# dylkot/cNMF

Measured on AMD Instinct MI355X. Metric: NMF restarts/sec (50000x2000xK5..13), higher is better.
Workload: dtype f32 (exact integer f16 plane x 2 f16 planes with per-row exponent, f32 accumulate)

## Files before the change

### cnmf_amd/csrc/kernels_gemm2h.hip.h

```cpp
#pragma once
#include <hip/hip_runtime.h>
#include "kernels_gemm3.hip.h"

namespace cnmf {

typedef _Float16 f16x8 __attribute__((ext_vector_type(8)));
typedef float f32x4_g __attribute__((ext_vector_type(4)));
#ifdef CNMF_G2_LDS_STORE
constexpr bool G2_LDS_STORE = true;
#else
constexpr bool G2_LDS_STORE = false;
#endif

constexpr int G2_ROWB = 64;
constexpr int G2_A = G3_MW * G2_ROWB;
constexpr int G2_B = G3C_JW * 32;
constexpr float G2_COUNT_BASE = 2048.0f;

constexpr int g2_imgs(int nsub) { return nsub == 1 ? 4 : 3; }
constexpr int g2_img_bytes(int nsub, bool with_hi) { return nsub * (G2_A + (with_hi ? 2 : 1) * G2_B); }
constexpr int g2_lds_bytes(int nsub, bool with_hi) { return g2_imgs(nsub) * g2_img_bytes(nsub, with_hi); }

__device__ __forceinline__ unsigned short f16_bits(float x)
{
    const _Float16 h = (_Float16)x;
    return __builtin_bit_cast(unsigned short, h);
}
__device__ __forceinline__ float f16_to_f32(unsigned short b) { return (float)__builtin_bit_cast(_Float16, b); }

__device__ __forceinline__ int g2_row_shift(float mx)
{
    if (!(mx > 0.f)) return 0;
    int e;
    frexpf(mx, &e);
    const int s = 15 - e;
    return s > 120 ? 120 : (s < -110 ? -110 : s);
}

__device__ __forceinline__ void split2h(float y, unsigned short& h, unsigned short& m)
{
    h = f16_bits(y);
    m = f16_bits(y - f16_to_f32(h));
}

struct SplitFused { const int* shift_in; int* shift_out; };
template <int TROWS, int TKB>
__device__ __forceinline__ void split2h_tiled_body(const float* __restrict__ src, int ld, int K, int TR,
                                                   unsigned short* __restrict__ dst, const double* __restrict__ kscale,
                                                   const float* __restrict__ rmax_part, int parts,
                                                   float* __restrict__ inv_scale, int bx, int nbx, int by,
                                                   unsigned short* tile_, float* red_, SplitFused fu = SplitFused{nullptr, nullptr})
{
    static_assert(TROWS * TKB == 256, "tile = 256 (row, block) pairs");
    constexpr int NQ = 256 / TROWS;
    constexpr int KQ = TKB * 4;
    constexpr int RPP = 256 / KQ;
    unsigned short (*tile)[TROWS][32] = reinterpret_cast<unsigned short (*)[TROWS][32]>(tile_);
    float (*red)[TROWS] = reinterpret_cast<float (*)[TROWS]>(red_);
    const int t = threadIdx.x;
    const int r0 = by * TROWS;
    const int kq = t % KQ, rr = t / KQ;
    const int ntiles = K / (16 * TKB);
    const bool fused = fu.shift_in != nullptr;
    float4 v[4];
    if (!fused) {
        const int k0 = bx * 16 * TKB;
#pragma unroll
        for (int i = 0; i < 4; ++i)
            v[i] = *reinterpret_cast<const float4*>(src + (size_t)(r0 + rr + RPP * i) * ld + k0 + kq * 4);
    }
    {
        const int row = t % TROWS, qt = t / TROWS;
        float mx = 0.f;
        for (int p0 = qt; p0 < parts; p0 += 8 * NQ) {
            float v[8];
#pragma unroll
            for (int j = 0; j < 8; ++j) v[j] = (p0 + j * NQ < parts) ? rmax_part[(size_t)(r0 + row) * parts + p0 + j * NQ] : 0.f;
#pragma unroll
            for (int j = 0; j < 8; ++j) mx = fmaxf(mx, v[j]);
        }
        red[qt][row] = mx;
    }
    __syncthreads();
    int sh[4];
    bool redo = false;
#pragma unroll
    for (int i = 0; i < 4; ++i) {
        const int row = rr + RPP * i;
        float mx = 0.f;
#pragma unroll
        for (int q = 0; q < NQ; ++q) mx = fmaxf(mx, red[q][row]);
        sh[i] = g2_row_shift(mx);
        if (fused) {
            const int su = fu.shift_in[r0 + row];
            const float ymax = ldexpf(mx, su);
            const bool ok = !(mx > 0.f) || (ymax < 60000.0f && ymax >= 1024.0f);
            const bool keep = !(mx > 0.f) || (ymax < 46340.0f && ymax >= 8192.0f);
            if (bx == 0 && kq == 0) fu.shift_out[r0 + row] = (ok && keep) ? su : sh[i];
            if (ok) sh[i] = su; else redo = true;
        }
        if (bx == 0 && kq == 0) inv_scale[r0 + row] = ldexpf(1.0f, -sh[i]);
    }
    if (fused) {
        if (!__syncthreads_or(redo ? 1 : 0)) return;
        const int k0 = bx * 16 * TKB;
#pragma unroll
        for (int i = 0; i < 4; ++i)
            v[i] = *reinterpret_cast<const float4*>(src + (size_t)(r0 + rr + RPP * i) * ld + k0 + kq * 4);
    }
    __syncthreads();
    const int Kb = K / 16;
    const int tr = r0 / TR, rin = r0 % TR;
    for (int kt = bx; kt < ntiles; kt += nbx) {
        const int k0 = kt * 16 * TKB;
        float4 vn[4];
        const bool has_next = kt + nbx < ntiles;
        if (has_next) {
#pragma unroll
            for (int i = 0; i < 4; ++i)
                vn[i] = *reinterpret_cast<const float4*>(src + (size_t)(r0 + rr + RPP * i) * ld + (k0 + nbx * 16 * TKB) + kq * 4);
        }
#pragma unroll
        for (int i = 0; i < 4; ++i) {
            const int row = rr + RPP * i;
            float x[4] = {v[i].x, v[i].y, v[i].z, v[i].w};
            if (kscale) {
#pragma unroll
                for (int e = 0; e < 4; ++e) x[e] = (float)((double)x[e] * kscale[k0 + kq * 4 + e]);
            }
            unsigned short p[2][4];
#pragma unroll
            for (int e = 0; e < 4; ++e) split2h(ldexpf(x[e], sh[i]), p[0][e], p[1][e]);
            const int hf = (kq >> 1) & 1, swz = (row >> 2) & 3;
#pragma unroll
            for (int q = 0; q < 2; ++q) {
                uint2 w;
                w.x = p[q][0] | ((unsigned)p[q][1] << 16); w.y = p[q][2] | ((unsigned)p[q][3] << 16);
                *reinterpret_cast<uint2*>(&tile[kq >> 2][row][((2 * q + hf) ^ swz) * 8 + (kq & 1) * 4]) = w;
            }
        }
        __syncthreads();
#pragma unroll
        for (int pass = 0; pass < 4; ++pass) {
            const int c = pass * 256 + t;
            const int b = c / (TROWS * 4), within = c % (TROWS * 4);
            unsigned short* g = dst + (((size_t)tr * Kb + (k0 / 16 + b)) * TR + rin) * 32;
            reinterpret_cast<u32x4*>(g)[within] = reinterpret_cast<const u32x4*>(&tile[b][0][0])[within];
        }
        __syncthreads();
        if (has_next) {
#pragma unroll
            for (int i = 0; i < 4; ++i) v[i] = vn[i];
        }
    }
}

template <int TROWS, int TKB>
__global__ __launch_bounds__(256) void split2h_tiled_kernel(const float* __restrict__ src, int ld, int K, int TR,
                                                            unsigned short* __restrict__ dst,
                                                            const double* __restrict__ kscale,
                                                            const float* __restrict__ rmax_part, int parts,
                                                            float* __restrict__ inv_scale)
{
    __shared__ __attribute__((aligned(16))) unsigned short tile[256 * 32];
    float* red = reinterpret_cast<float*>(tile);
    split2h_tiled_body<TROWS, TKB>(src, ld, K, TR, dst, kscale, rmax_part, parts, inv_scale, blockIdx.x, gridDim.x,
                                   blockIdx.y, tile, red);
}

__global__ __launch_bounds__(256) void rowmax_part_kernel(const float* __restrict__ V, int ld, int L, int span,
                                                          const double* __restrict__ kscale, int parts,
                                                          float* __restrict__ rmax_part)
{
    const int row = blockIdx.y * 4 + (threadIdx.x >> 6), lane = threadIdx.x & 63, p = blockIdx.x;
    const int j0 = p * span, j1 = min(L, j0 + span);
    float mx = 0.f;
    for (int j = j0 + lane; j < j1; j += 64) {
        float x = V[(size_t)row * ld + j];
        if (kscale) x = (float)((double)x * kscale[j]);
        mx = fmaxf(mx, x);
    }
#pragma unroll
    for (int o = 32; o > 0; o >>= 1) mx = fmaxf(mx, __shfl_xor(mx, o, 64));
    if (lane == 0) rmax_part[(size_t)row * parts + p] = mx;
}

__device__ __forceinline__ void count_lo_hi_2048(float n, float& lo, float& hi)
{
    if (n <= G2_COUNT_BASE) { lo = n; hi = 0.f; }
    else { hi = floorf(n * (1.0f / G2_COUNT_BASE)); lo = n - G2_COUNT_BASE * hi; hi *= G2_COUNT_BASE; }
}

__device__ __forceinline__ void store_plane_row_swz(unsigned short* d, const unsigned short* p, int row_in_tile)
{
    const int swz = (row_in_tile >> 3) & 1;
#pragma unroll
    for (int hf = 0; hf < 2; ++hf) {
        u32x4 w;
        w.x = p[8 * hf + 0] | ((unsigned)p[8 * hf + 1] << 16); w.y = p[8 * hf + 2] | ((unsigned)p[8 * hf + 3] << 16);
        w.z = p[8 * hf + 4] | ((unsigned)p[8 * hf + 5] << 16); w.w = p[8 * hf + 6] | ((unsigned)p[8 * hf + 7] << 16);
        *reinterpret_cast<u32x4*>(d + (hf ^ swz) * 8) = w;
    }
}

__global__ __launch_bounds__(256) void count_planes_f16_kernel(const float* __restrict__ X, int ld, int N, int G,
                                                               int rows_pad, int K, int TR,
                                                               const float* __restrict__ unit,
                                                               unsigned short* __restrict__ dst,
                                                               unsigned short* __restrict__ dst_hi,
                                                               unsigned int* __restrict__ hiflag)
{
    const long long t = (long long)blockIdx.x * 256 + threadIdx.x;
    const int Kb = K / 16;
    if (t >= (long long)rows_pad * Kb) return;
    const int row = (int)(t / Kb), kb = (int)(t % Kb);
    unsigned short p[16], ph[16];
    bool any_hi = false;
#pragma unroll
    for (int i = 0; i < 16; ++i) {
        const int g = kb * 16 + i;
        float n = 0.f, lo, hi;
        if (row < N && g < G) { const float u = unit[g]; if (u > 0.f) n = rintf(X[(size_t)row * ld + g] / u); }
        count_lo_hi_2048(n, lo, hi);
        p[i] = f16_bits(lo); ph[i] = f16_bits(hi);
        any_hi |= hi != 0.f;
    }
    const size_t blk = (size_t)(row / TR) * Kb + kb;
    store_plane_row_swz(dst + (blk * TR + (row % TR)) * 16, p, row % TR);
    if (dst_hi) {
        store_plane_row_swz(dst_hi + (blk * TR + (row % TR)) * 16, ph, row % TR);
        if (any_hi) atomicOr(&hiflag[(size_t)(row / TR) * ((Kb + 31) / 32) + (kb >> 5)], 1u << (kb & 31));
    }
}

__global__ __launch_bounds__(256) void count_planes_f16_transpose_kernel(const float* __restrict__ X, int ld, int N, int G,
                                                                         int rows_pad, int K, int TR,
                                                                         const float* __restrict__ unit,
                                                                         unsigned short* __restrict__ dst,
                                                                         unsigned short* __restrict__ dst_hi,
                                                                         unsigned int* __restrict__ hiflag)
{
    const int j = blockIdx.y * 256 + threadIdx.x;
    const int kb = blockIdx.x;
    if (j >= rows_pad) return;
    const int Kb = K / 16;
    const float u = (j < G) ? unit[j] : 0.f;
    unsigned short p[16], ph[16];
    bool any_hi = false;
#pragma unroll
    for (int i = 0; i < 16; ++i) {
        const int c = kb * 16 + i;
        float n = 0.f, lo, hi;
        if (u > 0.f && c < N) n = rintf(X[(size_t)c * ld + j] / u);
        count_lo_hi_2048(n, lo, hi);
        p[i] = f16_bits(lo); ph[i] = f16_bits(hi);
        any_hi |= hi != 0.f;
    }
    const size_t blk = (size_t)(j / TR) * Kb + kb;
    store_plane_row_swz(dst + (blk * TR + (j % TR)) * 16, p, j % TR);
    if (dst_hi) {
        store_plane_row_swz(dst_hi + (blk * TR + (j % TR)) * 16, ph, j % TR);
        if (any_hi) atomicOr(&hiflag[(size_t)(j / TR) * ((Kb + 31) / 32) + (kb >> 5)], 1u << (kb & 31));
    }
}

__global__ __launch_bounds__(256) void x2h_rowshift_kernel(const float* __restrict__ X, int ld, int N, int G,
                                                           int transpose, int rows_pad, int* __restrict__ shift,
                                                           float* __restrict__ inv_scale)
{
    if (!transpose) {
        const int row = blockIdx.x * 4 + (threadIdx.x >> 6), lane = threadIdx.x & 63;
        if (row >= rows_pad) return;
        float mx = 0.f;
        if (row < N) for (int g = lane; g < G; g += 64) mx = fmaxf(mx, X[(size_t)row * ld + g]);
#pragma unroll
        for (int o = 32; o > 0; o >>= 1) mx = fmaxf(mx, __shfl_xor(mx, o, 64));
        if (lane == 0) { const int s = g2_row_shift(mx); shift[row] = s; inv_scale[row] = ldexpf(1.0f, -s); }
    } else {
        const int g = blockIdx.x * 256 + threadIdx.x;
        if (g >= rows_pad) return;
        float mx = 0.f;
        if (g < G) for (int r = 0; r < N; ++r) mx = fmaxf(mx, X[(size_t)r * ld + g]);
        const int s = g2_row_shift(mx);
        shift[g] = s; inv_scale[g] = ldexpf(1.0f, -s);
    }
}

__global__ __launch_bounds__(256) void x2h_planes_kernel(const float* __restrict__ X, int ld, int N, int G, int rows_pad,
                                                         int K, int TR, const int* __restrict__ shift,
                                                         unsigned short* __restrict__ dst_h, unsigned short* __restrict__ dst_m)
{
    const long long t = (long long)blockIdx.x * 256 + threadIdx.x;
    const int Kb = K / 16;
    if (t >= (long long)rows_pad * Kb) return;
    const int row = (int)(t / Kb), kb = (int)(t % Kb);
    const int s = shift[row];
    unsigned short ph[16], pm[16];
#pragma unroll
    for (int i = 0; i < 16; ++i) {
        const int g = kb * 16 + i;
        const float x = (row < N && g < G) ? X[(size_t)row * ld + g] : 0.f;
        split2h(ldexpf(x, s), ph[i], pm[i]);
    }
    const size_t blk = (size_t)(row / TR) * Kb + kb;
    store_plane_row_swz(dst_h + (blk * TR + (row % TR)) * 16, ph, row % TR);
    store_plane_row_swz(dst_m + (blk * TR + (row % TR)) * 16, pm, row % TR);
}

__global__ __launch_bounds__(256) void x2h_planes_transpose_kernel(const float* __restrict__ X, int ld, int N, int G,
                                                                   int rows_pad, int K, int TR,
                                                                   const int* __restrict__ shift,
                                                                   unsigned short* __restrict__ dst_h,
                                                                   unsigned short* __restrict__ dst_m)
{
    const int j = blockIdx.y * 256 + threadIdx.x;
    const int kb = blockIdx.x;
    if (j >= rows_pad) return;
    const int Kb = K / 16;
    const int s = shift[j];
    unsigned short ph[16], pm[16];
#pragma unroll
    for (int i = 0; i < 16; ++i) {
        const int c = kb * 16 + i;
        const float x = (j < G && c < N) ? X[(size_t)c * ld + j] : 0.f;
        split2h(ldexpf(x, s), ph[i], pm[i]);
    }
    const size_t blk = (size_t)(j / TR) * Kb + kb;
    store_plane_row_swz(dst_h + (blk * TR + (j % TR)) * 16, ph, j % TR);
    store_plane_row_swz(dst_m + (blk * TR + (j % TR)) * 16, pm, j % TR);
}

__global__ __launch_bounds__(256) void count_max_base_kernel(const float* __restrict__ X, int ld, int N, int G,
                                                             const float* __restrict__ unit, float base,
                                                             unsigned* __restrict__ any_big)
{
    const int g = blockIdx.x * 256 + threadIdx.x;
    if (g >= G) return;
    const float u = unit[g];
    if (u <= 0.f) return;
    const int r0 = blockIdx.y * 256, r1 = min(N, r0 + 256);
    bool big = false;
    for (int r = r0; r < r1; ++r) big |= rintf(X[(size_t)r * ld + g] / u) > base;
    if (big) atomicOr(any_big, 1u);
}

struct G2NoEpi { static constexpr bool enabled = false; };
template <int NSUB, bool HI, int VAR = 0, bool NTB = true, bool PART = false, bool GEN = false, class EPI = G2NoEpi>
__device__ __forceinline__ void gemm2h_segment(const unsigned char* __restrict__ A2, const unsigned char* __restrict__ B1,
                                               const unsigned char* __restrict__ Bhi,
                                               const unsigned int* __restrict__ hiflag,
                                               const float* __restrict__ rscale,
                                               int Kb, float* __restrict__ C, int ldc, int m0, int j0, int kb0,
                                               int nkb, unsigned char* smem, const float* __restrict__ cscale = nullptr,
                                               unsigned live = 0xffu, const EPI* epi = nullptr, bool whole_tile = false)
{
    constexpr int IMGS = g2_imgs(NSUB);
    constexpr int IMG = g2_img_bytes(NSUB, HI);
    constexpr int OFF_B = NSUB * G2_A;
    constexpr int OFF_H = OFF_B + NSUB * G2_B;
    constexpr int NA = NSUB * 2, NB = NSUB;
    constexpr int NDMA = NA + NB;
    const int tid = threadIdx.x;
    const int lane = tid & 63, wave = tid >> 6;
    const int grp = wave >> 2, wn = wave & 3;
    const int li = lane & 31, h = lane >> 5;
    const int nst = nkb / NSUB;
    const unsigned lv = PART ? (unsigned)__builtin_amdgcn_readfirstlane((int)((live >> (grp * 4)) & 0xfu)) : 0xfu;
#define G2_LIVE(m_) (!PART || ((lv >> (m_)) & 1u))

    const size_t jblk = ((size_t)(j0 / G3C_JW) * Kb + kb0);
    const unsigned char* abase = A2 + ((size_t)(m0 / G3_MW) * Kb + kb0) * G2_A + tid * 16;
    const unsigned char* bbase = B1 + jblk * G2_B + tid * 16;
    const unsigned char* hbase = HI ? Bhi + jblk * G2_B + tid * 16 : nullptr;
    unsigned int fw[5] = {0u, 0u, 0u, 0u, 0u};
    if (HI) {
        const int KW = (Kb + 31) >> 5, w0 = kb0 >> 5;
        const unsigned int* fr = hiflag + (size_t)(j0 / G3C_JW) * KW;
#pragma unroll
        for (int w = 0; w < 5; ++w)
            fw[w] = (nkb > 129) ? 0xFFFFFFFFu : ((w0 + w < KW) ? __builtin_amdgcn_readfirstlane(fr[w0 + w]) : 0u);
    }
    const int fbit0 = kb0 & 31;

    f32x16_3 acc[4][2];
#pragma unroll
    for (int m = 0; m < 4; ++m)
#pragma unroll
        for (int n = 0; n < 2; ++n)
#pragma unroll
            for (int r = 0; r < 16; ++r) acc[m][n][r] = 0.f;

    const int a_row = (grp * 128 + li) * G2_ROWB;
    const int a_s0 = ((0 + h) ^ ((li >> 2) & 3)) * 16, a_s1 = ((2 + h) ^ ((li >> 2) & 3)) * 16;
    const int b_off = OFF_B + (wn * 64 + li) * 32 + (h ^ ((li >> 3) & 1)) * 16;

#define G2_BLKFLAG(b_) (HI && ((fw[(fbit0 + (b_)) >> 5 > 4 ? 4 : (fbit0 + (b_)) >> 5] >> ((fbit0 + (b_)) & 31)) & 1u))
#define G2_ISSUE(s_)                                                                               \
    {                                                                                              \
        unsigned char* d_ = smem + ((s_) % IMGS) * IMG + wave * 1024;                              \
        const unsigned char* a_ = abase + (size_t)(s_) * (NSUB * G2_A);                            \
        _Pragma("unroll") for (int i = 0; i < NA; ++i)                                             \
            __builtin_amdgcn_global_load_lds(G3_AS1(a_ + i * 8192), G3_AS3(d_ + i * 8192), 16, 0, 0); \
                                        \
        _Pragma("unroll") for (int i = 0; i < NB; ++i)                                             \
            __builtin_amdgcn_global_load_lds(G3_AS1(bbase + (size_t)(s_) * (NSUB * G2_B) + i * 8192), \
                                             G3_AS3(d_ + OFF_B + i * 8192), 16, 0, NTB ? 2 : 0);   \
        if (HI) {                                                                                  \
            _Pragma("unroll") for (int i = 0; i < NB; ++i)                                         \
                if (G2_BLKFLAG((s_) * NSUB + i))                                                   \
                    __builtin_amdgcn_global_load_lds(G3_AS1(hbase + (size_t)(s_) * (NSUB * G2_B) + i * 8192), \
                                                     G3_AS3(d_ + OFF_H + i * 8192), 16, 0, NTB ? 2 : 0); \
        }                                                                                          \
    }
#define G2_FRAG(ptr_) __builtin_bit_cast(f16x8, *reinterpret_cast<const u32x4*>(ptr_))
#define G2_READ(s_)                                                                                \
    {                                                                                              \
        const unsigned char* bb = smem + ((s_) % IMGS) * IMG;                                      \
        _Pragma("unroll") for (int u = 0; u < NSUB; ++u) {                                         \
            _Pragma("unroll") for (int n = 0; n < 2; ++n) bq[u][n] = G2_FRAG(bb + b_off + u * G2_B + n * 32 * 32); \
            if (HI) { _Pragma("unroll") for (int n = 0; n < 2; ++n)                                \
                          bh[u][n] = G2_FRAG(bb + b_off + NSUB * G2_B + u * G2_B + n * 32 * 32); } \
            _Pragma("unroll") for (int m = 0; m < 4; ++m) {                                        \
                aq[u][m][0] = G2_FRAG(bb + u * G2_A + a_row + m * 32 * G2_ROWB + a_s0);            \
                aq[u][m][1] = G2_FRAG(bb + u * G2_A + a_row + m * 32 * G2_ROWB + a_s1);            \
            }                                                                                      \
        }                                                                                          \
        __builtin_amdgcn_sched_barrier(0);                                                         \
    }
#define G2_MFMA(b_, u_, m_, q_)                                                                    \
    if (G2_LIVE(m_)) {                                                                             \
    acc[m_][0] = __builtin_amdgcn_mfma_f32_32x32x16_f16(aq[u_][m_][q_], b_[u_][0], acc[m_][0], 0, 0, 0); \
    acc[m_][1] = __builtin_amdgcn_mfma_f32_32x32x16_f16(aq[u_][m_][q_], b_[u_][1], acc[m_][1], 0, 0, 0); }
#define G2_MFMA4(b_, u_, ma_, mb_)                                                                 \
    G2_MFMA(b_, u_, ma_, 1) G2_MFMA(b_, u_, mb_, 1) G2_MFMA(b_, u_, ma_, 0) G2_MFMA(b_, u_, mb_, 0)
#define G2_MFMA2H(b_, u_, ma_, mb_) G2_MFMA(b_, u_, ma_, 0) G2_MFMA(b_, u_, mb_, 0)
#define G2_HALF(ma_, mb_)                                                                          \
    _Pragma("unroll") for (int u = 0; u < NSUB; ++u) {                                             \
        G2_MFMA4(bq, u, ma_, mb_)                                                                  \
        if (HI) { if (hi_blk[u]) { if constexpr (GEN) { G2_MFMA2H(bh, u, ma_, mb_) } else { G2_MFMA4(bh, u, ma_, mb_) } } } \
    }
#define G2_WAIT_AHEAD(cnt_)                                                                        \
    {                                                                                              \
        if constexpr ((cnt_) * NDMA == 0) G3_WAIT_VM(0);                                           \
        else if constexpr ((cnt_) * NDMA == 3) G3_WAIT_VM(3);                                      \
        else if constexpr ((cnt_) * NDMA == 6) G3_WAIT_VM(6);                                      \
        else if constexpr ((cnt_) * NDMA == 12) G3_WAIT_VM(12);                                    \
        else G3_WAIT_VM(0);                                                                        \
    }

    f16x8 bq[NSUB][2], bh[NSUB][2], aq[NSUB][4][2];
    constexpr int AHEAD = IMGS - 1;
    constexpr bool SPREAD = VAR >= 1 && NSUB == 2 && !HI;
    constexpr bool SPREADG = VAR >= 1 && NSUB == 1 && ((HI && GEN) || !HI);
    constexpr bool PRIO = false;
    constexpr bool NOMFMA = VAR == 2, NODMA = VAR == 3 || VAR == 6 || VAR == 7, SPLITRD = VAR >= 4;
    static_assert(VAR != 1 && VAR != 5, "instruction streams 1 and 5 were retired");
    constexpr bool NOREAD = VAR == 6 || VAR == 7;
    constexpr bool NOBAR = VAR == 7;
    G3_WAIT_VM(0);
    G2_ISSUE(0)
    if (nst > 1) G2_ISSUE(1)
    if (AHEAD > 2 && nst > 2) G2_ISSUE(2)
    if (AHEAD > 2 && nst > 2) G2_WAIT_AHEAD(2) else if (nst > 1) G2_WAIT_AHEAD(1) else G2_WAIT_AHEAD(0)
    if (grp == 1) G3_RAW_BARRIER()
    if constexpr (SPREADG) {
        static_assert(!SPREADG || (IMGS == 4 && NA == 2 && NB == 1), "one-block spread stream: four images, pieces A0 A1 B (Bhi)");
#define G2G_PIECE(s_, i_)                                                                          \
        {                                                                                          \
            unsigned char* d_ = smem + ((s_) % IMGS) * IMG + wave * 1024;                          \
            if ((i_) < NA)                                                                         \
                __builtin_amdgcn_global_load_lds(G3_AS1(abase + (size_t)(s_) * G2_A + (i_) * 8192), \
                                                 G3_AS3(d_ + (i_) * 8192), 16, 0, 0);              \
            else if ((i_) == NA)                                                                   \
                __builtin_amdgcn_global_load_lds(G3_AS1(bbase + (size_t)(s_) * G2_B), G3_AS3(d_ + OFF_B), 16, 0, NTB ? 2 : 0); \
            else if constexpr (HI)                                                                 \
                __builtin_amdgcn_global_load_lds(G3_AS1(hbase + (size_t)(s_) * G2_B), G3_AS3(d_ + OFF_H), 16, 0, NTB ? 2 : 0); \
            __builtin_amdgcn_sched_barrier(0);                                                     \
        }
#define G2G_READ_A(s_)                                                                             \
        {                                                                                          \
            const unsigned char* bb = smem + ((s_) % IMGS) * IMG;                                  \
            _Pragma("unroll") for (int n = 0; n < 2; ++n) bq[0][n] = G2_FRAG(bb + b_off + n * 32 * 32); \
            _Pragma("unroll") for (int m = 0; m < 2; ++m) {                                        \
                aq[0][m][1] = G2_FRAG(bb + a_row + m * 32 * G2_ROWB + a_s1);                       \
                aq[0][m][0] = G2_FRAG(bb + a_row + m * 32 * G2_ROWB + a_s0);                       \
            }                                                                                      \
            if constexpr (HI) { _Pragma("unroll") for (int n = 0; n < 2; ++n) bh[0][n] = G2_FRAG(bb + b_off + G2_B + n * 32 * 32); } \
            __builtin_amdgcn_sched_barrier(0);                                                     \
        }
#define G2G_READ_B(s_)                                                                             \
        {                                                                                          \
            const unsigned char* bb = smem + ((s_) % IMGS) * IMG;                                  \
            _Pragma("unroll") for (int m = 2; m < 4; ++m) {                                        \
                aq[0][m][1] = G2_FRAG(bb + a_row + m * 32 * G2_ROWB + a_s1);                       \
                aq[0][m][0] = G2_FRAG(bb + a_row + m * 32 * G2_ROWB + a_s0);                       \
            }                                                                                      \
            __builtin_amdgcn_sched_barrier(0);                                                     \
        }
#define G2G_STEP(MORE_)                                                                            \
        {                                                                                          \
            G3_RAW_BARRIER()                                         \
            G2G_READ_A(s)                                                                          \
            G2_MFMA(bq, 0, 0, 1) G2_MFMA(bq, 0, 1, 1)                                              \
            if (MORE_) G2G_PIECE(s + AHEAD, 0)                                                     \
            G2_MFMA(bq, 0, 0, 0) G2_MFMA(bq, 0, 1, 0)                                              \
            G2G_READ_B(s)                                                                          \
            if (MORE_) G2G_PIECE(s + AHEAD, 1)                                                     \
            if constexpr (HI) { G2_MFMA(bh, 0, 0, 0) G2_MFMA(bh, 0, 1, 0) }                        \
            asm volatile("s_waitcnt lgkmcnt(0)" ::: "memory");                                     \
             \
            if (s + 1 < nst) { if (MORE_) { if constexpr (HI) G3_WAIT_VM(6); else G3_WAIT_VM(5); } else G3_WAIT_VM(0); } \
            G3_RAW_BARRIER()                                                              \
            G2_MFMA(bq, 0, 2, 1) G2_MFMA(bq, 0, 3, 1)                                              \
            if (MORE_) G2G_PIECE(s + AHEAD, 2)                                                     \
            G2_MFMA(bq, 0, 2, 0) G2_MFMA(bq, 0, 3, 0)                                              \
            if constexpr (HI) { if (MORE_) G2G_PIECE(s + AHEAD, 3)                                 \
                                G2_MFMA(bh, 0, 2, 0) G2_MFMA(bh, 0, 3, 0) }                        \
        }
        {
            int s = 0;
            const int n_main = nst - AHEAD;
            for (; s < n_main; ++s) G2G_STEP(true)
            for (; s < nst; ++s) G2G_STEP(false)
        }
#undef G2G_STEP
#undef G2G_READ_B
#undef G2G_READ_A
#undef G2G_PIECE
    } else if constexpr (!SPREAD) {
        for (int s = 0; s < nst; ++s) {
            bool hi_blk[NSUB];
#pragma unroll
            for (int u = 0; u < NSUB; ++u) hi_blk[u] = G2_BLKFLAG(s * NSUB + u);
            G3_RAW_BARRIER()
            if (s + AHEAD < nst) G2_ISSUE(s + AHEAD)
            G2_READ(s)
            if (PRIO) __builtin_amdgcn_s_setprio(1);
            G2_HALF(0, 1)
            if (PRIO) __builtin_amdgcn_s_setprio(0);
            asm volatile("s_waitcnt lgkmcnt(0)" ::: "memory");
            if (s + 1 < nst) {
                if (AHEAD > 2 && s + 3 < nst) G2_WAIT_AHEAD(2) else if (s + 2 < nst) G2_WAIT_AHEAD(1) else G2_WAIT_AHEAD(0)
            }
            G3_RAW_BARRIER()
            if (PRIO) __builtin_amdgcn_s_setprio(1);
            G2_HALF(2, 3)
            if (PRIO) __builtin_amdgcn_s_setprio(0);
        }
    } else {
#define G2_PIECE(s_, i_)                                                                           \
        {                                                                                          \
            unsigned char* d_ = smem + ((s_) % IMGS) * IMG + wave * 1024;                          \
            if ((i_) < NA)                                                                         \
                __builtin_amdgcn_global_load_lds(G3_AS1(abase + (size_t)(s_) * (NSUB * G2_A) + (i_) * 8192), \
                                                 G3_AS3(d_ + (i_) * 8192), 16, 0, 0);              \
            else                                                                                   \
                __builtin_amdgcn_global_load_lds(G3_AS1(bbase + (size_t)(s_) * (NSUB * G2_B) + ((i_) - NA) * 8192), \
                                                 G3_AS3(d_ + OFF_B + ((i_) - NA) * 8192), 16, 0, NTB ? 2 : 0); \
            __builtin_amdgcn_sched_barrier(0);                                                     \
        }
#define G2_MF(u_, m_, q_)                                                                          \
        if constexpr (NOMFMA) { asm volatile("" :: "v"(aq[u_][m_][q_]), "v"(bq[u_][0]), "v"(bq[u_][1])); }        \
        else { G2_MFMA(bq, u_, m_, q_) }
#define G2_READ_A(s_)                                                                              \
    {                                                                                              \
        const unsigned char* bb = smem + ((s_) % IMGS) * IMG;                                      \
        _Pragma("unroll") for (int u = 0; u < NSUB; ++u) {                                         \
            _Pragma("unroll") for (int n = 0; n < 2; ++n) bq[u][n] = G2_FRAG(bb + b_off + u * G2_B + n * 32 * 32); \
            _Pragma("unroll") for (int m = 0; m < 2; ++m) {                                        \
                aq[u][m][1] = G2_FRAG(bb + u * G2_A + a_row + m * 32 * G2_ROWB + a_s1);            \
                aq[u][m][0] = G2_FRAG(bb + u * G2_A + a_row + m * 32 * G2_ROWB + a_s0);            \
            }                                                                                      \
        }                                                                                          \
        __builtin_amdgcn_sched_barrier(0);                                                         \
    }
#define G2_READ_B(s_)                                                                              \
    {                                                                                              \
        const unsigned char* bb = smem + ((s_) % IMGS) * IMG;                                      \
        _Pragma("unroll") for (int u = 0; u < NSUB; ++u)                                           \
            _Pragma("unroll") for (int m = 2; m < 4; ++m) {                                        \
                aq[u][m][1] = G2_FRAG(bb + u * G2_A + a_row + m * 32 * G2_ROWB + a_s1);            \
                aq[u][m][0] = G2_FRAG(bb + u * G2_A + a_row + m * 32 * G2_ROWB + a_s0);            \
            }                                                                                      \
        __builtin_amdgcn_sched_barrier(0);                                                         \
    }
#define G2_STEP(MORE_)                                                                             \
        {                                                                                          \
            if constexpr (!NOBAR) G3_RAW_BARRIER()                                        \
            if constexpr (NOREAD) { if (s == 0) { G2_READ(s) } }                                   \
            else if constexpr (SPLITRD) { G2_READ_A(s) } else { G2_READ(s) }                       \
            G2_MF(0, 0, 1) G2_MF(0, 1, 1)                                                          \
            if (MORE_) G2_PIECE(s + AHEAD, 0)                                                      \
            G2_MF(0, 0, 0) G2_MF(0, 1, 0)                                                          \
            if constexpr (SPLITRD && !NOREAD) { G2_READ_B(s) }                                     \
            if (MORE_) G2_PIECE(s + AHEAD, 1)                                                      \
            G2_MF(1, 0, 1) G2_MF(1, 1, 1)                                                          \
            if (MORE_) G2_PIECE(s + AHEAD, 2)                                                      \
            G2_MF(1, 0, 0) G2_MF(1, 1, 0)                                                          \
            asm volatile("s_waitcnt lgkmcnt(0)" ::: "memory");                                     \
             \
            if (s + 1 < nst) { if (MORE_) G3_WAIT_VM(3); else G3_WAIT_VM(0); }                     \
            if constexpr (!NOBAR) G3_RAW_BARRIER()                                        \
            G2_MF(0, 2, 1) G2_MF(0, 3, 1)                                                          \
            if (MORE_) G2_PIECE(s + AHEAD, 3)                                                      \
            G2_MF(0, 2, 0) G2_MF(0, 3, 0)                                                          \
            if (MORE_) G2_PIECE(s + AHEAD, 4)                                                      \
            G2_MF(1, 2, 1) G2_MF(1, 3, 1)                                                          \
            if (MORE_) G2_PIECE(s + AHEAD, 5)                                                      \
            G2_MF(1, 2, 0) G2_MF(1, 3, 0)                                                          \
        }
        {
            int s = 0;
            const int n_main = NODMA ? 0 : nst - AHEAD;
            for (; s < n_main; ++s) G2_STEP(true)
            for (; s < nst; ++s) G2_STEP(false)
        }
#undef G2_STEP
#undef G2_READ_B
#undef G2_READ_A
#undef G2_MF
#undef G2_PIECE
    }
    if (grp == 0) G3_RAW_BARRIER()
#undef G2_WAIT_AHEAD
#undef G2_HALF
#undef G2_MFMA2H
#undef G2_MFMA4
#undef G2_MFMA
#undef G2_READ
#undef G2_FRAG
#undef G2_ISSUE
#undef G2_BLKFLAG

    if constexpr (EPI::enabled) {
        if (whole_tile && epi->on) { (*epi)(acc, rscale, C, ldc, m0, j0, smem); return; }
    }
    if (C == nullptr) return;
    const int j = j0 + wn * 64 + li;
    const float cs[2] = {(HI && cscale) ? cscale[j] : 1.0f, (HI && cscale) ? cscale[j + 32] : 1.0f};
    if constexpr (!PART && G2_LDS_STORE && g2_lds_bytes(NSUB, HI) >= 8 * 16384) {
        float* tw = reinterpret_cast<float*>(smem) + wave * 4096;
#pragma unroll
        for (int mp = 0; mp < 2; ++mp) {
#pragma unroll
            for (int mm = 0; mm < 2; ++mm) {
                const int m = 2 * mp + mm;
#pragma unroll
                for (int n = 0; n < 2; ++n)
#pragma unroll
                    for (int r = 0; r < 16; ++r) {
                        const int rl = 4 * h + (r & 3) + 8 * (r >> 2);
                        tw[(mm * 32 + rl) * 64 + n * 32 + li] = (acc[m][n][r] * rscale[m0 + grp * 128 + m * 32 + rl]) * cs[n];
                    }
            }
            __builtin_amdgcn_wave_barrier();
#pragma unroll
            for (int i = 0; i < 16; ++i) {
                const int c = 4 * i + (lane >> 4);
                const f32x4_g v = *reinterpret_cast<const f32x4_g*>(tw + c * 64 + 4 * (lane & 15));
                *reinterpret_cast<f32x4_g*>(C + (size_t)(m0 + grp * 128 + mp * 64 + c) * ldc + j0 + wn * 64 + 4 * (lane & 15)) = v;
            }
            __builtin_amdgcn_wave_barrier();
        }
    } else {
#pragma unroll
    for (int m = 0; m < 4; ++m) {
        if (!G2_LIVE(m)) continue;
        const int cbase = m0 + grp * 128 + m * 32 + 4 * h;
#pragma unroll
        for (int n = 0; n < 2; ++n)
#pragma unroll
            for (int r = 0; r < 16; ++r) {
                const int row = cbase + (r & 3) + 8 * (r >> 2);
                C[(size_t)row * ldc + j + n * 32] = (acc[m][n][r] * rscale[row]) * cs[n];
            }
    }
    }
#undef G2_LIVE
}

template <int NSUB, bool HI, int VAR = 0, bool PART = false, bool GEN = false>
__global__ __launch_bounds__(512) void gemm2h_kernel(const unsigned char* __restrict__ A2,
                                                     const unsigned char* __restrict__ B1,
                                                     const unsigned char* __restrict__ Bhi,
                                                     const unsigned int* __restrict__ hiflag,
                                                     const float* __restrict__ rscale, int Kb,
                                                     float* __restrict__ C, int ldc, long long c_split_stride,
                                                     int kb_per, const float* __restrict__ cscale = nullptr,
                                                     unsigned long long livemask = ~0ull)
{
    extern __shared__ __attribute__((aligned(16))) unsigned char smem3[];
    int jt = blockIdx.x, mg = blockIdx.y, z = blockIdx.z;
    if ((gridDim.z & 7) == 0) {
        const int L = blockIdx.x + (int)gridDim.x * (blockIdx.y + (int)gridDim.y * blockIdx.z);
        const int xcd = L & 7, idx = L >> 3;
        jt = idx % (int)gridDim.x;
        mg = (idx / (int)gridDim.x) % (int)gridDim.y;
        z = xcd + 8 * (idx / (int)(gridDim.x * gridDim.y));
    }
    const int kb0 = z * kb_per;
    const int nkb = min(kb_per, Kb - kb0);
    gemm2h_segment<NSUB, HI, VAR, true, PART, GEN>(A2, B1, Bhi, hiflag, rscale, Kb, C ? C + (size_t)z * c_split_stride : nullptr, ldc, mg * G3_MW,
                                              jt * G3C_JW, kb0, nkb, smem3, cscale, (unsigned)((livemask >> (8 * mg)) & 0xffu));
}

template <int NSUB, bool HI, int VAR = 0, bool NTB = true, bool PART = false, bool GEN = false, class EPI = G2NoEpi>
__global__ __launch_bounds__(512) void gemm2h_streamk_kernel(const unsigned char* __restrict__ A2,
                                                             const unsigned char* __restrict__ B1,
                                                             const unsigned char* __restrict__ Bhi,
                                                             const unsigned int* __restrict__ hiflag,
                                                             const float* __restrict__ rscale, int Kb,
                                                             float* __restrict__ C0, float* __restrict__ C1,
                                                             float* __restrict__ C2, int ldc, int MG, int T, int xmap,
                                                             const float* __restrict__ cscale = nullptr,
                                                             unsigned long long livemask = ~0ull, EPI epi = EPI{})
{
    extern __shared__ __attribute__((aligned(16))) unsigned char smem3[];
    const int Ks = Kb / NSUB;
    const long long U = (long long)T * Ks;
    const int P = (int)gridDim.x;
    const int q = (xmap && MG > 1 && P % MG == 0) ? ((int)blockIdx.x % MG) * (P / MG) + (int)blockIdx.x / MG : (int)blockIdx.x;
    long long u = U * q / P;
    const long long u1 = U * (q + 1) / P;
    const int NJ = T / MG;
    while (u < u1) {
        const int tile = (int)(u / Ks), ks = (int)(u % Ks);
        const int ke = (int)min((long long)Ks, ks + (u1 - u));
        const int mg = tile / NJ, jt = tile % NJ;
        gemm2h_segment<NSUB, HI, VAR, NTB, PART, GEN, EPI>(A2, B1, Bhi, hiflag, rscale, Kb, (ks == 0) ? C0 : (ke == Ks ? C1 : C2), ldc, mg * G3_MW,
                                                 jt * G3C_JW, ks * NSUB, (ke - ks) * NSUB, smem3, cscale,
                                                 (unsigned)((livemask >> (8 * mg)) & 0xffu), &epi, ks == 0 && ke == Ks);
        u += ke - ks;
        G3_WAIT_VM(0);
        __syncthreads();
    }
}

}
```

Before: 227.1.

## Route two-block gemm2h segments through a 16x16x32 MFMA body

Adds a dedicated NSUB=2 segment that merges the two k-blocks into one 64-deep step and uses 16x16x32 f16 MFMAs with 8x4 accumulator tiles instead of the older 32x32 instruction path. It removes the former spread stream and handles all two-block calls in the new body. With the default variant, the new body issues all six next-stage DMA pieces in one burst at the top of each step instead of interleaving them between MFMAs. The aim is higher matrix-core throughput and a simpler load schedule. The trade-offs are more accumulator registers and more fragment reads per step, and the HI plane and tile epilogue are no longer supported for two-block segments.

Result: faster. 232.1, median of 6 (+2.2%).

```diff
diff --git a/cnmf_amd/csrc/kernels_gemm2h.hip.h b/cnmf_amd/csrc/kernels_gemm2h.hip.h
--- a/cnmf_amd/csrc/kernels_gemm2h.hip.h
+++ b/cnmf_amd/csrc/kernels_gemm2h.hip.h
@@ -345,6 +345,149 @@
 }
 
 struct G2NoEpi { static constexpr bool enabled = false; };
+
+template <int VAR, bool NTB, bool PART>
+__device__ __forceinline__ void gemm2h_segment_mf16(const unsigned char* __restrict__ A2, const unsigned char* __restrict__ B1,
+                                                    const float* __restrict__ rscale, int Kb, float* __restrict__ C,
+                                                    int ldc, int m0, int j0, int kb0, int nkb, unsigned char* smem,
+                                                    unsigned live)
+{
+    static_assert(VAR == 0 || VAR == 2 || VAR == 3 || VAR == 4 || VAR == 6 || VAR == 7, "instruction streams 1 and 5 were retired");
+    constexpr int NSUB = 2, IMGS = g2_imgs(NSUB), IMG = g2_img_bytes(NSUB, false);
+    constexpr int OFF_B = NSUB * G2_A;
+    constexpr int NA = NSUB * 2, NB = NSUB, AHEAD = IMGS - 1;
+    constexpr bool BURST = VAR == 0, NOMFMA = VAR == 2, NODMA = VAR == 3 || VAR == 6 || VAR == 7;
+    constexpr bool NOREAD = VAR == 6 || VAR == 7, NOBAR = VAR == 7;
+    static_assert(IMGS == 3 && NA + NB == 6, "three images, six pieces per step");
+    const int tid = threadIdx.x;
+    const int lane = tid & 63, wave = tid >> 6;
+    const int grp = wave >> 2, wn = wave & 3;
+    const int r = lane & 15, g = lane >> 4;
+    const int ub = g >> 1, hf = g & 1;
+    const int nst = nkb / NSUB;
+    const unsigned lv = PART ? (unsigned)__builtin_amdgcn_readfirstlane((int)((live >> (grp * 4)) & 0xfu)) : 0xfu;
+#define G2_LIVE(mt_) (!PART || ((lv >> ((mt_) >> 1)) & 1u))
+
+    const unsigned char* abase = A2 + ((size_t)(m0 / G3_MW) * Kb + kb0) * G2_A + tid * 16;
+    const unsigned char* bbase = B1 + ((size_t)(j0 / G3C_JW) * Kb + kb0) * G2_B + tid * 16;
+
+    f32x4_g acc[8][4];
+#pragma unroll
+    for (int mt = 0; mt < 8; ++mt)
+#pragma unroll
+        for (int nt = 0; nt < 4; ++nt)
+#pragma unroll
+            for (int i = 0; i < 4; ++i) acc[mt][nt][i] = 0.f;
+
+    const int a_row = ub * G2_A + (grp * 128 + r) * G2_ROWB;
+    const int a_s0 = ((0 + hf) ^ ((r >> 2) & 3)) * 16, a_s1 = ((2 + hf) ^ ((r >> 2) & 3)) * 16;
+    const int b_off = OFF_B + ub * G2_B + (wn * 64 + r) * 32 + (hf ^ ((r >> 3) & 1)) * 16;
+
+#define G2_PIECE(s_, i_)                                                                           \
+    {                                                                                              \
+        unsigned char* d_ = smem + ((s_) % IMGS) * IMG + wave * 1024;                              \
+        if ((i_) < NA)                                                                             \
+            __builtin_amdgcn_global_load_lds(G3_AS1(abase + (size_t)(s_) * (NSUB * G2_A) + (i_) * 8192), \
+                                             G3_AS3(d_ + (i_) * 8192), 16, 0, 0);                  \
+        else                              \
+            __builtin_amdgcn_global_load_lds(G3_AS1(bbase + (size_t)(s_) * (NSUB * G2_B) + ((i_) - NA) * 8192), \
+                                             G3_AS3(d_ + OFF_B + ((i_) - NA) * 8192), 16, 0, NTB ? 2 : 0); \
+        __builtin_amdgcn_sched_barrier(0);                                                         \
+    }
+#define G2_ISSUE(s_) { _Pragma("unroll") for (int i = 0; i < NA + NB; ++i) G2_PIECE(s_, i) }
+#define G2_FRAG(ptr_) __builtin_bit_cast(f16x8, *reinterpret_cast<const u32x4*>(ptr_))
+#define G2_AFRAG(bb_, mt_, q_) G2_FRAG((bb_) + a_row + (mt_) * 16 * G2_ROWB + ((q_) ? a_s1 : a_s0))
+#define G2_READ_A(s_)                                                                              \
+    {                                                                                              \
+        const unsigned char* bb = smem + ((s_) % IMGS) * IMG;                                      \
+        _Pragma("unroll") for (int nt = 0; nt < 4; ++nt) bq[nt] = G2_FRAG(bb + b_off + nt * 16 * 32); \
+        _Pragma("unroll") for (int mp = 0; mp < 4; mp += 2) {                                      \
+            aq[mp][1] = G2_AFRAG(bb, mp, 1); aq[mp + 1][1] = G2_AFRAG(bb, mp + 1, 1);              \
+            aq[mp][0] = G2_AFRAG(bb, mp, 0); aq[mp + 1][0] = G2_AFRAG(bb, mp + 1, 0);              \
+        }                                                                                          \
+        __builtin_amdgcn_sched_barrier(0);                                                         \
+    }
+#define G2_READ_B(s_)                                                                              \
+    {                                                                                              \
+        const unsigned char* bb = smem + ((s_) % IMGS) * IMG;                                      \
+        _Pragma("unroll") for (int mp = 4; mp < 8; mp += 2) {                                      \
+            aq[mp][1] = G2_AFRAG(bb, mp, 1); aq[mp + 1][1] = G2_AFRAG(bb, mp + 1, 1);              \
+            aq[mp][0] = G2_AFRAG(bb, mp, 0); aq[mp + 1][0] = G2_AFRAG(bb, mp + 1, 0);              \
+        }                                                                                          \
+        __builtin_amdgcn_sched_barrier(0);                                                         \
+    }
+#define G2_MF(mt_, q_)                                                                             \
+    if constexpr (NOMFMA) { asm volatile("" :: "v"(aq[mt_][q_]), "v"(bq[0]), "v"(bq[1]), "v"(bq[2]), "v"(bq[3])); } \
+    else if (G2_LIVE(mt_)) {                                                                       \
+        _Pragma("unroll") for (int nt = 0; nt < 4; ++nt)                                           \
+            acc[mt_][nt] = __builtin_amdgcn_mfma_f32_16x16x32_f16(aq[mt_][q_], bq[nt], acc[mt_][nt], 0, 0, 0); \
+    }
+#define G2_MF8(ma_, mb_, q_) G2_MF(ma_, q_) G2_MF(mb_, q_)
+#define G2_STEP(MORE_)                                                                             \
+    {                                                                                              \
+        if constexpr (!NOBAR) G3_RAW_BARRIER()                   \
+        if (BURST && MORE_) G2_ISSUE(s + AHEAD)                                                    \
+        if constexpr (NOREAD) { if (s == 0) { G2_READ_A(s) G2_READ_B(s) } } else { G2_READ_A(s) }  \
+        G2_MF8(0, 1, 1)                                                                            \
+        if (!BURST && MORE_) G2_PIECE(s + AHEAD, 0)                                                \
+        G2_MF8(0, 1, 0)                                                                            \
+        if constexpr (!NOREAD) { G2_READ_B(s) }                                                    \
+        if (!BURST && MORE_) G2_PIECE(s + AHEAD, 1)                                                \
+        G2_MF8(2, 3, 1)                                                                            \
+        if (!BURST && MORE_) G2_PIECE(s + AHEAD, 2)                                                \
+        G2_MF8(2, 3, 0)                                                                            \
+        asm volatile("s_waitcnt lgkmcnt(0)" ::: "memory");       \
+         \
+        if (s + 1 < nst) { if (MORE_) { if constexpr (BURST) G3_WAIT_VM(6); else G3_WAIT_VM(3); } else G3_WAIT_VM(0); } \
+        if constexpr (!NOBAR) G3_RAW_BARRIER()                                            \
+        G2_MF8(4, 5, 1)                                                                            \
+        if (!BURST && MORE_) G2_PIECE(s + AHEAD, 3)                                                \
+        G2_MF8(4, 5, 0)                                                                            \
+        if (!BURST && MORE_) G2_PIECE(s + AHEAD, 4)                                                \
+        G2_MF8(6, 7, 1)                                                                            \
+        if (!BURST && MORE_) G2_PIECE(s + AHEAD, 5)                                                \
+        G2_MF8(6, 7, 0)                                                                            \
+    }
+
+    f16x8 bq[4], aq[8][2];
+    G3_WAIT_VM(0);
+    G2_ISSUE(0)
+    if (nst > 1) G2_ISSUE(1)
+    if (nst > 1) G3_WAIT_VM(6); else G3_WAIT_VM(0);
+    if (grp == 1) G3_RAW_BARRIER()
+    {
+        int s = 0;
+        const int n_main = NODMA ? 0 : nst - AHEAD;
+        for (; s < n_main; ++s) G2_STEP(true)
+        for (; s < nst; ++s) G2_STEP(false)
+    }
+    if (grp == 0) G3_RAW_BARRIER()
+#undef G2_STEP
+#undef G2_MF8
+#undef G2_MF
+#undef G2_READ_B
+#undef G2_READ_A
+#undef G2_AFRAG
+#undef G2_FRAG
+#undef G2_ISSUE
+#undef G2_PIECE
+
+    if (C == nullptr) return;
+#pragma unroll
+    for (int mt = 0; mt < 8; ++mt) {
+        if (!G2_LIVE(mt)) continue;
+        const int row0 = m0 + grp * 128 + mt * 16 + 4 * g;
+#pragma unroll
+        for (int i = 0; i < 4; ++i) {
+            const float rs = rscale[row0 + i];
+#pragma unroll
+            for (int nt = 0; nt < 4; ++nt)
+                C[(size_t)(row0 + i) * ldc + j0 + wn * 64 + nt * 16 + r] = acc[mt][nt][i] * rs;
+        }
+    }
+#undef G2_LIVE
+}
+
 template <int NSUB, bool HI, int VAR = 0, bool NTB = true, bool PART = false, bool GEN = false, class EPI = G2NoEpi>
 __device__ __forceinline__ void gemm2h_segment(const unsigned char* __restrict__ A2, const unsigned char* __restrict__ B1,
                                                const unsigned char* __restrict__ Bhi,
@@ -354,6 +497,12 @@
                                                int nkb, unsigned char* smem, const float* __restrict__ cscale = nullptr,
                                                unsigned live = 0xffu, const EPI* epi = nullptr, bool whole_tile = false)
 {
+    static_assert(NSUB == 1 || !HI, "two blocks per step: one count plane only");
+    if constexpr (NSUB == 2) {
+        static_assert(!EPI::enabled, "the 16x16x32 body has no tile epilogue");
+        gemm2h_segment_mf16<VAR, NTB, PART>(A2, B1, rscale, Kb, C, ldc, m0, j0, kb0, nkb, smem, live);
+        return;
+    }
     constexpr int IMGS = g2_imgs(NSUB);
     constexpr int IMG = g2_img_bytes(NSUB, HI);
     constexpr int OFF_B = NSUB * G2_A;
@@ -450,13 +599,9 @@
 
     f16x8 bq[NSUB][2], bh[NSUB][2], aq[NSUB][4][2];
     constexpr int AHEAD = IMGS - 1;
-    constexpr bool SPREAD = VAR >= 1 && NSUB == 2 && !HI;
     constexpr bool SPREADG = VAR >= 1 && NSUB == 1 && ((HI && GEN) || !HI);
     constexpr bool PRIO = false;
-    constexpr bool NOMFMA = VAR == 2, NODMA = VAR == 3 || VAR == 6 || VAR == 7, SPLITRD = VAR >= 4;
     static_assert(VAR != 1 && VAR != 5, "instruction streams 1 and 5 were retired");
-    constexpr bool NOREAD = VAR == 6 || VAR == 7;
-    constexpr bool NOBAR = VAR == 7;
     G3_WAIT_VM(0);
     G2_ISSUE(0)
     if (nst > 1) G2_ISSUE(1)
@@ -527,7 +672,7 @@
 #undef G2G_READ_B
 #undef G2G_READ_A
 #undef G2G_PIECE
-    } else if constexpr (!SPREAD) {
+    } else {
         for (int s = 0; s < nst; ++s) {
             bool hi_blk[NSUB];
 #pragma unroll
@@ -547,79 +692,6 @@
             G2_HALF(2, 3)
             if (PRIO) __builtin_amdgcn_s_setprio(0);
         }
-    } else {
-#define G2_PIECE(s_, i_)                                                                           \
-        {                                                                                          \
-            unsigned char* d_ = smem + ((s_) % IMGS) * IMG + wave * 1024;                          \
-            if ((i_) < NA)                                                                         \
-                __builtin_amdgcn_global_load_lds(G3_AS1(abase + (size_t)(s_) * (NSUB * G2_A) + (i_) * 8192), \
-                                                 G3_AS3(d_ + (i_) * 8192), 16, 0, 0);              \
-            else                                                                                   \
-                __builtin_amdgcn_global_load_lds(G3_AS1(bbase + (size_t)(s_) * (NSUB * G2_B) + ((i_) - NA) * 8192), \
-                                                 G3_AS3(d_ + OFF_B + ((i_) - NA) * 8192), 16, 0, NTB ? 2 : 0); \
-            __builtin_amdgcn_sched_barrier(0);                                                     \
-        }
-#define G2_MF(u_, m_, q_)                                                                          \
-        if constexpr (NOMFMA) { asm volatile("" :: "v"(aq[u_][m_][q_]), "v"(bq[u_][0]), "v"(bq[u_][1])); }        \
-        else { G2_MFMA(bq, u_, m_, q_) }
-#define G2_READ_A(s_)                                                                              \
-    {                                                                                              \
-        const unsigned char* bb = smem + ((s_) % IMGS) * IMG;                                      \
-        _Pragma("unroll") for (int u = 0; u < NSUB; ++u) {                                         \
-            _Pragma("unroll") for (int n = 0; n < 2; ++n) bq[u][n] = G2_FRAG(bb + b_off + u * G2_B + n * 32 * 32); \
-            _Pragma("unroll") for (int m = 0; m < 2; ++m) {                                        \
-                aq[u][m][1] = G2_FRAG(bb + u * G2_A + a_row + m * 32 * G2_ROWB + a_s1);            \
-                aq[u][m][0] = G2_FRAG(bb + u * G2_A + a_row + m * 32 * G2_ROWB + a_s0);            \
-            }                                                                                      \
-        }                                                                                          \
-        __builtin_amdgcn_sched_barrier(0);                                                         \
-    }
-#define G2_READ_B(s_)                                                                              \
-    {                                                                                              \
-        const unsigned char* bb = smem + ((s_) % IMGS) * IMG;                                      \
-        _Pragma("unroll") for (int u = 0; u < NSUB; ++u)                                           \
-            _Pragma("unroll") for (int m = 2; m < 4; ++m) {                                        \
-                aq[u][m][1] = G2_FRAG(bb + u * G2_A + a_row + m * 32 * G2_ROWB + a_s1);            \
-                aq[u][m][0] = G2_FRAG(bb + u * G2_A + a_row + m * 32 * G2_ROWB + a_s0);            \
-            }                                                                                      \
-        __builtin_amdgcn_sched_barrier(0);                                                         \
-    }
-#define G2_STEP(MORE_)                                                                             \
-        {                                                                                          \
-            if constexpr (!NOBAR) G3_RAW_BARRIER()                                        \
-            if constexpr (NOREAD) { if (s == 0) { G2_READ(s) } }                                   \
-            else if constexpr (SPLITRD) { G2_READ_A(s) } else { G2_READ(s) }                       \
-            G2_MF(0, 0, 1) G2_MF(0, 1, 1)                                                          \
-            if (MORE_) G2_PIECE(s + AHEAD, 0)                                                      \
-            G2_MF(0, 0, 0) G2_MF(0, 1, 0)                                                          \
-            if constexpr (SPLITRD && !NOREAD) { G2_READ_B(s) }                                     \
-            if (MORE_) G2_PIECE(s + AHEAD, 1)                                                      \
-            G2_MF(1, 0, 1) G2_MF(1, 1, 1)                                                          \
-            if (MORE_) G2_PIECE(s + AHEAD, 2)                                                      \
-            G2_MF(1, 0, 0) G2_MF(1, 1, 0)                                                          \
-            asm volatile("s_waitcnt lgkmcnt(0)" ::: "memory");                                     \
-             \
-            if (s + 1 < nst) { if (MORE_) G3_WAIT_VM(3); else G3_WAIT_VM(0); }                     \
-            if constexpr (!NOBAR) G3_RAW_BARRIER()                                        \
-            G2_MF(0, 2, 1) G2_MF(0, 3, 1)                                                          \
-            if (MORE_) G2_PIECE(s + AHEAD, 3)                                                      \
-            G2_MF(0, 2, 0) G2_MF(0, 3, 0)                                                          \
-            if (MORE_) G2_PIECE(s + AHEAD, 4)                                                      \
-            G2_MF(1, 2, 1) G2_MF(1, 3, 1)                                                          \
-            if (MORE_) G2_PIECE(s + AHEAD, 5)                                                      \
-            G2_MF(1, 2, 0) G2_MF(1, 3, 0)                                                          \
-        }
-        {
-            int s = 0;
-            const int n_main = NODMA ? 0 : nst - AHEAD;
-            for (; s < n_main; ++s) G2_STEP(true)
-            for (; s < nst; ++s) G2_STEP(false)
-        }
-#undef G2_STEP
-#undef G2_READ_B
-#undef G2_READ_A
-#undef G2_MF
-#undef G2_PIECE
     }
     if (grp == 0) G3_RAW_BARRIER()
 #undef G2_WAIT_AHEAD
```
